# neuromodulation/PyPARRM

Hardware: NVIDIA B200
Metric: filter_data channel-samples/sec (higher is better)
Workload: dtype f64

## Files before the change

pyparrm_b200/csrc/filter.cu:

```cuda
#include <string.h>

#include "common.cuh"
#include "filter_jit.h"
#include "filter_plan.h"
#include "gather.cuh"

namespace parrm {

static thread_local const char* g_last_kernel = "";

template <typename T>
struct FilterArgs {
  const T* x;
  T* out;
  const int32_t* taps;
  int64_t ld_x, x_t0, n_x;
  int64_t ld_out, t0, n_out;
  int64_t n_total;
  int32_t n_taps, w_lo, w_hi;
  int32_t tile;
};

template <typename T>
__global__ void __launch_bounds__(kGatherThreads)
// ... 109 lines not shown
  filter_gather_smem_kernel<T><<<grid, kGatherThreads, smem, stream>>>(a);
  PARRM_LAUNCH_OK("filter_gather_smem_kernel");
  g_last_kernel = "filter_gather_smem_kernel";
  return PARRM_OK;
}


}

extern "C" {

const char* parrm_filter_last_kernel(void) { return parrm::g_last_kernel; }

int parrm_filter_specialise_check(const void* h_plan, int dtype,
                                  const parrm_filter_options_t* options, int32_t* shape,
                                  size_t* cubin_bytes) {
  using namespace parrm;
  PARRM_REQUIRE(h_plan != nullptr, "parrm_filter_specialise_check: null plan");
  const FilterPlanHeader* hdr = static_cast<const FilterPlanHeader*>(h_plan);
  PARRM_REQUIRE(hdr->magic == kPlanMagic && hdr->version == kPlanVersion,
                "parrm_filter_specialise_check: not a filter plan");
  const int32_t* h_terms = reinterpret_cast<const int32_t*>(
      static_cast<const unsigned char*>(h_plan) + hdr->terms_offset);
  FilterTuning tune{0, options ? options->steps_per_chunk : 0,
                    options ? options->prefetch_chunks : 0, options ? options->ctas_per_sm : 0,
                    options ? options->variant : 0, options ? options->timeline : 0};
  CombEShape s;
  if (!comb_e_shape(hdr, h_terms, dtype, &tune, &s)) {
    set_error("parrm_filter_specialise_check: this plan is outside the specialised kernel's range");
    return PARRM_ERR_UNSUPPORTED;
  }
  if (shape) {
    const int32_t v[12] = {s.d, s.nk, s.m[0], s.m[1], s.nb[0], s.nb[1], s.n_plus + s.n_minus,
                           s.u, s.pf, s.ctas, s.smem_bytes, ((s.d + 31) / 32) * 32 + 32};
    for (int i = 0; i < 12; ++i) shape[i] = v[i];
  }
  if (cubin_bytes == nullptr) return PARRM_OK;
  return comb_e_compile_only(s, cubin_bytes);
}

int parrm_filter_apply(const void* d_x, int64_t ld_x, int64_t x_t0, int64_t n_x, void* d_out,
                       int64_t ld_out, int64_t t0, int64_t n_out, int64_t n_samples_total,
                       int64_t n_chans, const void* d_plan, const void* h_plan, int dtype,
                       void* stream) {
  return parrm_filter_apply_ex(d_x, ld_x, x_t0, n_x, d_out, ld_out, t0, n_out, n_samples_total,
                               n_chans, d_plan, h_plan, dtype, nullptr, stream);
}

int parrm_filter_apply_ex(const void* d_x, int64_t ld_x, int64_t x_t0, int64_t n_x, void* d_out,
                          int64_t ld_out, int64_t t0, int64_t n_out, int64_t n_samples_total,
                          int64_t n_chans, const void* d_plan, const void* h_plan, int dtype,
                          const parrm_filter_options_t* options, void* stream) {
  PARRM_NVTX("parrm_filter_apply_ex");
  using namespace parrm;
  PARRM_REQUIRE(d_plan != nullptr && h_plan != nullptr, "parrm_filter_apply: null plan");
  const FilterPlanHeader* hdr = static_cast<const FilterPlanHeader*>(h_plan);
  PARRM_REQUIRE(hdr->magic == kPlanMagic && hdr->version == kPlanVersion,
                "parrm_filter_apply: not a filter plan");
  PARRM_REQUIRE(hdr->dtype == dtype, "parrm_filter_apply: plan built for another dtype");
  PARRM_REQUIRE(dtype == PARRM_F64 || dtype == PARRM_F32, "parrm_filter_apply: bad dtype %d", dtype);
  PARRM_REQUIRE(n_chans >= 0 && n_out >= 0 && n_x >= 0 && n_samples_total >= 0,
                "parrm_filter_apply: negative size");
  PARRM_REQUIRE(n_chans <= 65535, "parrm_filter_apply: more than 65535 channels per call");
  const int want = options ? options->kernel : PARRM_FILTER_KERNEL_AUTO;
  PARRM_REQUIRE(want == PARRM_FILTER_KERNEL_AUTO || want == PARRM_FILTER_KERNEL_GATHER ||
                    want == PARRM_FILTER_KERNEL_SPECIALISED,
                "parrm_filter_apply: unknown kernel choice %d", want);
// ... 101 lines not shown
```

pyparrm_b200/csrc/filter_comb_e.cuh:

```cuda
#pragma once

#ifdef __CUDACC_RTC__
typedef signed char int8_t;
typedef int int32_t;
typedef unsigned int uint32_t;
typedef long long int64_t;
typedef unsigned long long uint64_t;
typedef unsigned long long uintptr_t;
#else
#include <stdint.h>
#endif

#ifndef PE_D
#define PE_T double
#define PE_D 200
#define PE_NK 2
#define PE_M0 20
#define PE_M1 10
#define PE_NB0 7
#define PE_NB1 2
#define PE_OFF0 -1969, -1954, -1923, -1877, -1846, -1831, -1800
#define PE_OFF1 -1908, 108
#define PE_NPLUS 1
#define PE_PLUS -2000
#define PE_NMINUS 0
#define PE_MINUS 0
#define PE_CENTRE -1
#define PE_U 10
#define PE_PF 2
#define PE_NTAPS 160
#define PE_WLO -2000
#define PE_WHI 2000
#define PE_BACK 108
#define PE_FWD 2000
#define PE_CTAS 2
#endif
#ifndef PE_VARIANT
#define PE_VARIANT 0
#endif

namespace parrm_e {

typedef PE_T T;
typedef double T2;
constexpr int D = PE_D;
constexpr int NK = PE_NK;
constexpr int M0 = PE_M0;
constexpr int M1 = PE_M1;
constexpr int NB0 = PE_NB0;
constexpr int NB1 = PE_NB1;
constexpr int NPLUS = PE_NPLUS;
constexpr int NMINUS = PE_NMINUS;
constexpr int CENTRE = PE_CENTRE;
constexpr int U = PE_U;
constexpr int PF = PE_PF;
constexpr int NTAPS = PE_NTAPS;
constexpr int WLO = PE_WLO;
constexpr int WHI = PE_WHI;
constexpr int BACK = PE_BACK;
constexpr int FWD = PE_FWD;
constexpr int ES = int(sizeof(T));
constexpr int VEC = 16 / ES;
constexpr int CH = U * D;
constexpr int HB = (BACK + CH - 1) / CH;
constexpr int HF = (FWD + CH - 1) / CH;
constexpr int MIR = HB + HF;
constexpr int Q = HB + HF + 1 + PF;
constexpr int GPB = (M0 + U - 1) / U;
constexpr int B = GPB * U;
constexpr int NPG = GPB;
constexpr int NW = (D + 31) / 32;
constexpr int NT = NW * 32 + 32;
constexpr int BAR_BYTES = ((2 * Q * 8 + 127) / 128) * 128;
constexpr int SMEM_BYTES = BAR_BYTES + (Q + MIR) * CH * ES;
static_assert((CH * ES) % 16 == 0, "chunk must be a whole number of 16-byte units");
static_assert(M0 >= M1 && M0 >= 1, "box lengths ordered");

__host__ __device__ constexpr int off0(int b) {
  constexpr int t[NB0 > 0 ? NB0 : 1] = {PE_OFF0};
  return t[b];
}
__host__ __device__ constexpr int off1(int b) {
  constexpr int t[NB1 > 0 ? NB1 : 1] = {PE_OFF1};
  return t[b];
}
__host__ __device__ constexpr int plus_tap(int i) {
  constexpr int t[NPLUS > 0 ? NPLUS : 1] = {PE_PLUS};
  return t[i];
}
__host__ __device__ constexpr int minus_tap(int i) {
  constexpr int t[NMINUS > 0 ? NMINUS : 1] = {PE_MINUS};
  return t[i];
}

struct Args {
  const T* x;
  T* out;
  const int32_t* taps;
  const int32_t* count;
  const T2* recip;
  int64_t ld_x, x_t0, n_x;
  int64_t ld_out, t0, n_out;
  int64_t n_total;
  int64_t total_groups;
  int32_t groups_per_chan;
// ... 53 lines not shown
                                        T xc, T tot) {
  const int64_t v1 = min64(max64(t, WLO - 1), WHI);
  const int64_t v2 = min64(max64(t - n_total, WLO - 1), WHI);
  const int n_in = count[v1 - (WLO - 1)] - count[v2 - (WLO - 1)];
  T y = xc - tot * T(recip[n_in]);
  if (n_in == 0) y = T(0);
  return y;
}

__device__ __noinline__ T direct_value(const int32_t* __restrict__ taps,
                                       const T2* __restrict__ recip, int64_t n_total, T t_max,
                                       const T* __restrict__ xrow, int64_t t, int64_t lo_valid,
                                       int64_t hi_valid) {
  T acc = T(0);
  int n_in = 0;
  for (int k = 0; k < NTAPS; ++k) {
    const int64_t g = t - taps[k];
    if (g < 0 || g >= n_total) continue;
    ++n_in;
    if (g >= lo_valid && g < hi_valid) acc += xrow[g];
  }
  if (n_in == 0) return T(0);
  const T y = xrow[t] - acc * T(recip[n_in]);
  return fabs(y) <= t_max ? y : T(0);
}

struct Walk {
  int pb;
  int rslot;
  int fslot;
  uint32_t fphase;
};

__device__ __forceinline__ void group_begin(Walk& w, uint32_t bars) {
  mbar_wait(bars + w.fslot * 8, w.fphase);
  if (++w.fslot == Q) {
    w.fslot = 0;
    w.fphase ^= 1u;
  }
}
__device__ __forceinline__ void group_end(Walk& w, uint32_t bars, int lane, unsigned wmask) {
  __syncwarp(wmask);
  if (lane == 0) {
    asm volatile("mbarrier.arrive.shared::cta.b64 _, [%0];" ::"r"(bars + (Q + w.rslot) * 8)
                 : "memory");
  }
  w.pb += CH * ES;
  if (++w.rslot == Q) {
    w.rslot = 0;
    w.pb -= Q * CH * ES;
  }
}

struct Rings {
  T r0[B];
  T r1[NK > 1 ? B : 1];
  T S0, S1;
};

__device__ __forceinline__ T ring_sum0(const Rings& r, int s) {
  T a = r.r0[s];
#pragma unroll
  for (int i = 1; i < M0; ++i) a += r.r0[(s + B - i) % B];
  return a;
}
__device__ __forceinline__ T ring_sum1(const Rings& r, int s) {
  if (NK < 2) return T(0);
  T a = r.r1[s];
#pragma unroll
  for (int i = 1; i < M1; ++i) a += r.r1[(s + B - i) % B];
  return a;
}

template <bool FAST>
__device__ __forceinline__ int run_block(Rings& r, Walk& w, const Args& a,
                                         const unsigned char* const smem, uint32_t bars,
                                         int lane, unsigned wmask, int c, T* const orow,
                                         int& bad_lo, int& bad_hi, int64_t Tb, int g,
                                         int n_groups) {
  const T neg_inv_n = a.neg_inv_n;
  const T t_max = a.t_max;
  T* const op = orow + Tb + c;
  int done = 0;
#pragma unroll
  for (int gi = 0; gi < GPB; ++gi) {
    if (!FAST && g + gi >= n_groups) break;
    group_begin(w, bars);
    int mode = 1;
    if (!FAST) {
      const int64_t Tn = Tb + int64_t(gi) * CH;
      const bool interior = (Tn - WHI >= 0) && (Tn + CH - WLO <= a.n_total);
      const bool all_out = (Tn >= a.t0) && (Tn + CH <= a.t0 + a.n_out);
      mode = (g + gi < NPG) ? 0 : ((interior && all_out) ? 1 : 2);
    }
    const unsigned char* const p = smem + w.pb;
#pragma unroll
    for (int js = 0; js < U; ++js) {
      const int s = gi * U + js;
      auto ld = [&](int off) {
        return *reinterpret_cast<const T*>(p + (HB * CH + js * D - off) * ES);
      };
      r.S0 -= r.r0[(s + B - M0) % B];
      if (NK > 1) r.S1 -= r.r1[(s + B - M1) % B];
      T e0 = ld(off0(0));
      if (NB0 > 1) {
        T e0b = ld(off0(1));
#pragma unroll
        for (int b = 2; b < NB0; ++b) {
          if (b & 1) e0b += ld(off0(b)); else e0 += ld(off0(b));
        }
        e0 += e0b;
      }
      r.r0[s] = e0;
      r.S0 += e0;
      T tot = r.S0;
      if (NK > 1) {
        T e1 = ld(off1(0));
        if (NB1 > 1) {
          T e1b = ld(off1(1));
#pragma unroll
          for (int b = 2; b < NB1; ++b) {
            if (b & 1) e1b += ld(off1(b)); else e1 += ld(off1(b));
          }
          e1 += e1b;
        }
        r.r1[s] = e1;
        r.S1 += e1;
        tot += r.S1;
      }
      T single = T(0);
      if (NPLUS > 0) {
        single = ld(plus_tap(0));
#pragma unroll
        for (int i = 1; i < NPLUS; ++i) single += ld(plus_tap(i));
      }
#pragma unroll
      for (int i = 0; i < NMINUS; ++i) single -= ld(minus_tap(i));
      const T xc = ld(0);
      if (CENTRE != 0) single = fma(T(CENTRE), xc, single);
      if (NPLUS > 0 || NMINUS > 0 || CENTRE != 0) tot += single;
      if (FAST) {
        T y = fma(tot, neg_inv_n, xc);
        if (__builtin_expect(!(fabs(y) <= t_max), 0)) {
          r.S0 = ring_sum0(r, s);
          r.S1 = ring_sum1(r, s);
          bad_lo = min(bad_lo, g * U + s);
          bad_hi = max(bad_hi, g * U + s);
          y = T(0);
        }
        op[s * D] = y;
      } else if (mode != 0) {
        const int64_t t = Tb + c + int64_t(s) * D;
        if (ES == 4 && mode == 2) {
          r.S0 = ring_sum0(r, s);
          r.S1 = ring_sum1(r, s);
          tot = r.S0;
          if (NK > 1) tot += r.S1;
          if (NPLUS > 0 || NMINUS > 0 || CENTRE != 0) tot += single;
        }
        T y = mode == 1 ? fma(tot, neg_inv_n, xc) : edge_value(a.count, a.recip, t, a.n_total, xc, tot);
        if (__builtin_expect(!(fabs(y) <= t_max), 0)) {
          r.S0 = ring_sum0(r, s);
          r.S1 = ring_sum1(r, s);
          bad_lo = min(bad_lo, g * U + s);
          bad_hi = max(bad_hi, g * U + s);
          y = T(0);
        }
        if (t >= a.t0 && t < a.t0 + a.n_out) op[s * D] = y;
      }
    }
    group_end(w, bars, lane, wmask);
    ++done;
  }
  return done;
}

extern "C" __global__ void __launch_bounds__(NT, PE_CTAS) parrm_filter_comb_e(const Args a) {
  extern __shared__ __align__(128) unsigned char smem_raw[];
  uint64_t* const full = reinterpret_cast<uint64_t*>(smem_raw);
  uint64_t* const empty = full + Q;
  T* const ring = reinterpret_cast<T*>(smem_raw + BAR_BYTES);
  const int tid = threadIdx.x;
  const int lane = tid & 31;
  const bool is_producer = tid >= NW * 32;

  if (tid == 0) {
    for (int s = 0; s < Q; ++s) {
      mbar_init(&full[s], 1);
      mbar_init(&empty[s], NW);
    }
    asm volatile("fence.mbarrier_init.release.cluster;" ::: "memory");
  }
  __syncthreads();

  const int64_t lo_valid = max64(0, a.x_t0);
  const int64_t hi_valid = min64(a.n_total, a.x_t0 + a.n_x);
#if PE_VARIANT & 2
  unsigned long long tl_start = 0, tl_pieces = 0;
  if (tid == 0) asm volatile("mov.u64 %0, %%globaltimer;" : "=l"(tl_start));
#endif
  const int gpc = a.groups_per_chan;
  const int vpc = gpc + a.edge_total;
  const int64_t G_begin = a.total_groups * int64_t(blockIdx.x) / int64_t(gridDim.x);
  const int64_t G_end = a.total_groups * int64_t(blockIdx.x + 1) / int64_t(gridDim.x);
  const uint32_t bars = smem_u32(smem_raw);

  int fslot = 0;
  uint32_t fphase = 0;
  int rslot = 0;

  for (int64_t G = G_begin; G < G_end;) {
    const int64_t chan = G / vpc;
    const int v0 = int(G - chan * vpc);
    const int v1 = int(min64(vpc, v0 + (G_end - G)));
    G += v1 - v0;
    const int s0 = min(max(v0 - a.edge_start, 0), gpc);
    const int s1 = min(max(v1 - a.edge_start, 0), gpc);
    if (s1 <= s0) continue;
    const T* const xrow = a.x + chan * a.ld_x - a.x_t0;
    T* const orow = a.out + chan * a.ld_out - a.t0;
    const int gamma = int((VEC - int((reinterpret_cast<uintptr_t>(xrow) / ES) % VEC)) % VEC);
    const int64_t j_first = floor_div(a.t0 - gamma, CH);
    const int64_t j_last = floor_div(a.t0 + a.n_out - 1 - gamma, CH);
    const int64_t n_first = j_first + s0;
    const int64_t n_end = min64(j_first + s1, j_last + 1);
    if (n_first >= n_end) continue;
#if PE_VARIANT & 2
    ++tl_pieces;
#endif
    const int n_groups = NPG + int(n_end - n_first);
    const int n_chunks = n_groups + HB + HF;
    const int64_t c_first = n_first - NPG - HB;

    if (is_producer) {
      for (int i = 0; i < n_chunks; ++i) {
        const int64_t g0 = gamma + (c_first + i) * int64_t(CH);
        T* const dst = ring + fslot * CH;
        mbar_wait(bars + (Q + fslot) * 8, fphase ^ 1u);
        if (g0 >= lo_valid && g0 + CH <= hi_valid) {
          if (lane == 0) {
            asm volatile("fence.proxy.async.shared::cta;" ::: "memory");
            const bool mirror = fslot < MIR;
            mbar_expect_tx(&full[fslot], uint32_t(CH * ES) * (mirror ? 2u : 1u));
            bulk_g2s(dst, xrow + g0, uint32_t(CH * ES), &full[fslot]);
            if (mirror) bulk_g2s(dst + Q * CH, xrow + g0, uint32_t(CH * ES), &full[fslot]);
          }
        } else {
          for (int e = lane; e < CH; e += 32) {
            const int64_t g = g0 + e;
            const T v = (g >= lo_valid && g < hi_valid) ? xrow[g] : T(0);
            dst[e] = v;
            if (fslot < MIR) dst[Q * CH + e] = v;
          }
          __syncwarp();
          if (lane == 0) mbar_arrive(&full[fslot]);
        }
        if (++fslot == Q) {
          fslot = 0;
          fphase ^= 1u;
        }
      }
      continue;
    }

    if (tid >= D) continue;
    const int c = tid;
    const unsigned wmask = (tid | 31) < D ? 0xffffffffu : ((1u << (D & 31)) - 1u);
    for (int i = 0; i < HB + HF; ++i) {
      mbar_wait(bars + fslot * 8, fphase);
      if (++fslot == Q) {
        fslot = 0;
        fphase ^= 1u;
      }
    }
    Rings r;
#pragma unroll
    for (int s = 0; s < B; ++s) r.r0[s] = T(0);
#pragma unroll
    for (int s = 0; s < (NK > 1 ? B : 1); ++s) r.r1[s] = T(0);
    const int64_t T0 = gamma + (n_first - NPG) * int64_t(CH);
    Walk w;
    w.pb = BAR_BYTES + (rslot * CH + c) * ES;
    w.rslot = rslot;
    w.fslot = fslot;
    w.fphase = fphase;
    int bad_lo = 1 << 30, bad_hi = -1;
    for (int g = 0; g < n_groups;) {
      const int64_t Tb = T0 + int64_t(g) * CH;
      r.S0 = ring_sum0(r, B - 1);
      r.S1 = ring_sum1(r, B - 1);
      const bool fast = g >= NPG && g + GPB <= n_groups && Tb - WHI >= 0 &&
                        Tb + int64_t(B) * D - WLO <= a.n_total && Tb >= a.t0 &&
                        Tb + int64_t(B) * D <= a.t0 + a.n_out;
      if (fast) {
        g += run_block<true>(r, w, a, smem_raw, bars, lane, wmask, c, orow, bad_lo, bad_hi,
                             Tb, g, n_groups);
      } else {
        g += run_block<false>(r, w, a, smem_raw, bars, lane, wmask, c, orow, bad_lo, bad_hi,
                              Tb, g, n_groups);
      }
    }
    rslot = w.rslot;
    fslot = w.fslot;
    fphase = w.fphase;
    for (int k = bad_lo; k <= bad_hi; ++k) {
      const int64_t t = T0 + c + int64_t(k) * D;
      if (t >= a.t0 && t < a.t0 + a.n_out)
        orow[t] = direct_value(a.taps, a.recip, a.n_total, a.t_max, xrow, t, lo_valid, hi_valid);
    }
    __syncwarp(wmask);
    for (int i = 0; i < HB + HF; ++i) {
      if (lane == 0) mbar_arrive(&empty[rslot]);
      if (++rslot == Q) rslot = 0;
    }
  }
#if PE_VARIANT & 2
  if (tid == 0 && a.timeline) {
    unsigned long long tl_end;
    unsigned smid;
    asm volatile("mov.u64 %0, %%globaltimer;" : "=l"(tl_end));
    asm volatile("mov.u32 %0, %%smid;" : "=r"(smid));
    a.timeline[4 * blockIdx.x + 0] = smid;
    a.timeline[4 * blockIdx.x + 1] = tl_start;
    a.timeline[4 * blockIdx.x + 2] = tl_end;
    a.timeline[4 * blockIdx.x + 3] = tl_pieces;
  }
#endif
}

}
```

pyparrm_b200/csrc/filter_jit.cu:

```cuda
#include <cuda.h>
#include <dlfcn.h>
#include <string.h>

#include <algorithm>
#include <map>
#include <mutex>
#include <string>
#include <vector>

#include "common.cuh"
#include "filter_jit.h"
#include "filter_plan.h"

namespace parrm {
namespace {

const char kCombESource[] =
#include "filter_comb_e_src.inc"
    ;

typedef struct _nvrtcProgram* nvrtcProgram;
struct Nvrtc {
  void* handle = nullptr;
  int (*CreateProgram)(nvrtcProgram*, const char*, const char*, int, const char* const*,
// ... 150 lines not shown
    const int64_t ch = int64_t(u) * s.d;
    const int64_t hb = (s.back + ch - 1) / ch, hf = (s.fwd + ch - 1) / ch;
    const int64_t q = hb + hf + 1 + pf;
    return ((2 * q * 8 + 127) / 128) * 128 + (q + hb + hf) * ch * s.es;
  };
  auto usable = [&](int u) {
    return u >= 1 && (int64_t(u) * s.d * s.es) % 16 == 0 && (s.m[0] + u - 1) / u * u <= 64;
  };
  for (int ctas = ctas_first; ctas >= 1; --ctas) {
    const int64_t budget = int64_t(227) * 1024 / ctas - 1024;
    int u = 0;
    if (tune && tune->steps_per_chunk > 0) {
      u = tune->steps_per_chunk;
      if (!usable(u) || smem_for(u, pf_min) > budget) u = 0;
    } else {
      for (int cand = s.m[0]; cand >= 1 && u == 0; --cand)
        if (s.m[0] % cand == 0 && int64_t(cand) * s.d * s.es <= 32768 &&
            int64_t(cand) * s.d >= 512 && usable(cand) && smem_for(cand, pf_min) <= budget)
          u = cand;
      const int u_hi = int(std::max<int64_t>(1, 20480 / (int64_t(s.d) * s.es)));
      for (int cand = u_hi; cand >= 1 && u == 0; --cand)
        if (usable(cand) && smem_for(cand, pf_min) <= budget) u = cand;
      for (int cand = 1; cand <= 64 && u == 0; ++cand)
        if (usable(cand) && smem_for(cand, pf_min) <= budget) u = cand;
    }
    if (u == 0) continue;
    int pf = pf_min;
    while (pf < pf_max && smem_for(u, pf + 1) <= budget) ++pf;
    s.smem_bytes = int(smem_for(u, pf));
    s.ctas = ctas;
    s.u = u;
    s.pf = pf;
    s.variant = tune ? tune->variant : 0;
    *out = s;
    return true;
  }
  return false;
}

static int compile_cubin(const CombEShape& s, std::vector<char>* cubin) {
  Nvrtc* n = nvrtc();
  if (!n->ok) {
    const char* why = dlerror();
    set_error("parrm filter: NVRTC (libnvrtc.so.12) could not be opened: %s", why ? why : "?");
    return PARRM_ERR_UNSUPPORTED;
  }
  std::vector<std::string> opts = {
      "--gpu-architecture=sm_100a", "-std=c++17", "-lineinfo",
      std::string("-DPE_T=") + (s.es == 8 ? "double" : "float"),
      "-DPE_D=" + std::to_string(s.d), "-DPE_NK=" + std::to_string(s.nk),
      "-DPE_M0=" + std::to_string(s.m[0]), "-DPE_M1=" + std::to_string(s.m[1]),
      "-DPE_NB0=" + std::to_string(s.nb[0]), "-DPE_NB1=" + std::to_string(s.nb[1]),
      "-DPE_OFF0=" + join(s.off[0], s.nb[0]), "-DPE_OFF1=" + join(s.off[1], s.nb[1]),
      "-DPE_NPLUS=" + std::to_string(s.n_plus), "-DPE_PLUS=" + join(s.plus, s.n_plus),
      "-DPE_NMINUS=" + std::to_string(s.n_minus), "-DPE_MINUS=" + join(s.minus, s.n_minus),
      "-DPE_CENTRE=" + std::to_string(s.centre), "-DPE_U=" + std::to_string(s.u),
      "-DPE_PF=" + std::to_string(s.pf), "-DPE_NTAPS=" + std::to_string(s.n_taps),
      "-DPE_WLO=" + std::to_string(s.w_lo), "-DPE_WHI=" + std::to_string(s.w_hi),
      "-DPE_BACK=" + std::to_string(s.back), "-DPE_FWD=" + std::to_string(s.fwd),
      "-DPE_CTAS=" + std::to_string(s.ctas), "-DPE_VARIANT=" + std::to_string(s.variant)};
  std::vector<const char*> copts;
  for (const std::string& o : opts) copts.push_back(o.c_str());
  nvrtcProgram prog = nullptr;
  int rc = n->CreateProgram(&prog, kCombESource, "filter_comb_e.cu", 0, nullptr, nullptr);
  if (rc != 0) {
    set_error("nvrtcCreateProgram: %s", n->GetErrorString(rc));
    return PARRM_ERR_CUDA;
  }
  rc = n->CompileProgram(prog, int(copts.size()), copts.data());
  if (rc != 0) {
    size_t log_size = 0;
    n->GetProgramLogSize(prog, &log_size);
    std::string log(log_size + 1, '\0');
    if (log_size) n->GetProgramLog(prog, &log[0]);
    set_error("nvrtcCompileProgram: %s\n%.380s", n->GetErrorString(rc), log.c_str());
    n->DestroyProgram(&prog);
    return PARRM_ERR_CUDA;
  }
  size_t cubin_size = 0;
  n->GetCUBINSize(prog, &cubin_size);
  cubin->resize(cubin_size);
  rc = n->GetCUBIN(prog, cubin->data());
  n->DestroyProgram(&prog);
  if (rc != 0 || cubin_size == 0) {
    set_error("nvrtcGetCUBIN: %s", n->GetErrorString(rc));
    return PARRM_ERR_CUDA;
  }
  return PARRM_OK;
}

int comb_e_compile_only(const CombEShape& s, size_t* cubin_bytes) {
  std::vector<char> cubin;
  const int rc = compile_cubin(s, &cubin);
  if (rc == PARRM_OK && cubin_bytes) *cubin_bytes = cubin.size();
  return rc;
}

static int build_kernel(const CombEShape& s, Kernel* out) {
  Driver* d = driver();
  if (!d->ok) {
    set_error("parrm filter: CUDA driver entry points unavailable");
    return PARRM_ERR_UNSUPPORTED;
  }
  std::vector<char> cubin;
  const int rc = compile_cubin(s, &cubin);
  if (rc != PARRM_OK) return rc;
  PARRM_CUDA_OK(cudaFree(nullptr));
  CUmodule mod = nullptr;
  CUresult cr = d->ModuleLoadData(&mod, cubin.data());
  if (cr != CUDA_SUCCESS) return driver_fail(cr, "cuModuleLoadData");
  Kernel k;
  cr = d->ModuleGetFunction(&k.fn, mod, "parrm_filter_comb_e");
  if (cr != CUDA_SUCCESS) return driver_fail(cr, "cuModuleGetFunction");
  k.smem_bytes = s.smem_bytes;
  k.threads = ((s.d + 31) / 32) * 32 + 32;
  k.ctas_per_sm = s.ctas;
  k.chunk = s.u * s.d;
  k.priming_groups = (s.m[0] + s.u - 1) / s.u;
  cr = d->FuncSetAttribute(k.fn, CU_FUNC_ATTRIBUTE_MAX_DYNAMIC_SHARED_SIZE_BYTES, k.smem_bytes);
  if (cr != CUDA_SUCCESS) return driver_fail(cr, "cuFuncSetAttribute(max dynamic shared memory)");
  d->FuncSetAttribute(k.fn, CU_FUNC_ATTRIBUTE_PREFERRED_SHARED_MEMORY_CARVEOUT, 100);
  d->FuncGetAttribute(&k.regs, CU_FUNC_ATTRIBUTE_NUM_REGS, k.fn);
  *out = k;
  return PARRM_OK;
}

bool comb_e_cached(const CombEShape& s) {
  int dev = 0;
  if (cudaGetDevice(&dev) != cudaSuccess) return false;
  const std::string key = comb_e_key(s, dev);
  std::lock_guard<std::mutex> lock(g_mutex);
  return g_cache.count(key) != 0;
}

std::string comb_e_key(const CombEShape& s, int dev) {
  std::string key = std::to_string(dev) + "|" + std::to_string(s.es) + "|" + std::to_string(s.d) +
                    "|" + std::to_string(s.nk) + "|" + std::to_string(s.m[0]) + "|" +
                    std::to_string(s.m[1]) + "|" + join(s.off[0], s.nb[0]) + "|" +
                    join(s.off[1], s.nb[1]) + "|" + join(s.plus, s.n_plus) + "|" +
                    join(s.minus, s.n_minus) + "|" + std::to_string(s.centre) + "|" +
                    std::to_string(s.u) + "|" + std::to_string(s.pf) + "|" +
                    std::to_string(s.n_taps) + "|" + std::to_string(s.w_lo) + "|" +
                    std::to_string(s.w_hi) + "|" + std::to_string(s.ctas) + "|" +
                    std::to_string(s.variant);
  return key;
}

int launch_comb_e(const CombEShape& s, const void* d_x, void* d_out, const int32_t* d_taps,
                  const int32_t* d_count, const double* d_recip,
                  int64_t ld_x, int64_t x_t0, int64_t n_x, int64_t ld_out, int64_t t0,
                  int64_t n_out, int64_t n_total, int64_t n_chans, cudaStream_t stream,
                  int* regs_out, unsigned long long timeline) {
  int dev = 0;
  PARRM_CUDA_OK(cudaGetDevice(&dev));
  const std::string key = comb_e_key(s, dev);
  Kernel k;
  {
    std::lock_guard<std::mutex> lock(g_mutex);
    auto it = g_cache.find(key);
    if (it == g_cache.end()) {
      const int rc = build_kernel(s, &k);
      if (rc != PARRM_OK) return rc;
      g_cache[key] = k;
    } else {
      k = it->second;
    }
  }
  if (regs_out) *regs_out = k.regs;
  struct Args {
    const void* x;
    void* out;
    const int32_t* taps;
    const int32_t* count;
    const double* recip;
    int64_t ld_x, x_t0, n_x, ld_out, t0, n_out, n_total, total_groups;
    int32_t groups_per_chan, edge_start, edge_total, pad;
    unsigned long long timeline;
// ... 35 lines not shown
```

pyparrm_b200/csrc/filter_jit.h:

```cpp
#pragma once
#include <cuda_runtime.h>
#include <stdint.h>

#include <string>

#include "filter_plan.h"

namespace parrm {

struct FilterTuning {
  int kernel;
  int steps_per_chunk;
  int prefetch_chunks;
  int ctas_per_sm;
  int variant;
  unsigned long long timeline;
};

struct CombEShape {
  int es;
  int d, nk, m[2], nb[2];
  const int32_t* off[2];
  int n_plus, n_minus;
  const int32_t *plus, *minus;
  int centre, n_taps, w_lo, w_hi, back, fwd;
  int u, pf, ctas, smem_bytes, variant;
};

bool comb_e_shape(const FilterPlanHeader* hdr, const int32_t* terms, int dtype,
                  const FilterTuning* tune, CombEShape* out);
std::string comb_e_key(const CombEShape& s, int dev);
bool comb_e_cached(const CombEShape& s);
int comb_e_compile_only(const CombEShape& s, size_t* cubin_bytes);
int launch_comb_e(const CombEShape& s, const void* d_x, void* d_out, const int32_t* d_taps,
                  const int32_t* d_count, const double* d_recip,
                  int64_t ld_x, int64_t x_t0, int64_t n_x, int64_t ld_out, int64_t t0,
                  int64_t n_out, int64_t n_total, int64_t n_chans, cudaStream_t stream,
                  int* regs_out, unsigned long long timeline = 0);

}
```

pyparrm_b200/csrc/filter_plan.cu:

```cuda
#include <algorithm>
#include <string.h>
#include <vector>

#include "common.cuh"
#include "filter_plan.h"

namespace parrm {
namespace {

struct CombPlan {
  int d = 0, nk = 0;
  int m[kMaxBoxKinds] = {0, 0};
  std::vector<int> box[kMaxBoxKinds];
  std::vector<int> plus, minus;
  int centre = 0;
  double cost = 1e30;
  int n_terms() const { return int(box[0].size() + box[1].size() + plus.size() + minus.size()); }
};

bool cover(const std::vector<uint8_t>& bit, int lo, int hi, int d, int nk, const int* m,
           CombPlan* out) {
  const int span = hi - lo + 1;
  CombPlan p;
  p.d = d;
// ... 127 lines not shown
    std::vector<int> cand;
    auto add_len = [&](int len) {
      if (len >= 2 && len <= max_ring && std::find(cand.begin(), cand.end(), len) == cand.end())
        cand.push_back(len);
    };
    for (size_t i = 0; i < lengths.size() && i < 6; ++i) add_len(lengths[i].second);
    for (size_t i = 0; i < lengths.size() && i < 3 && cand.size() < 8; ++i) {
      const int len = lengths[i].second;
      if (len > max_ring || 2 * len > max_ring) {
        add_len((len + 1) / 2);
        add_len((len + 2) / 3);
      }
    }
    const int n_len = int(cand.size());
    for (int i = 0; i < n_len; ++i) {
      for (int j = i; j < n_len; ++j) {
        int m[2] = {cand[i], cand[j]};
        if (i != j && m[0] + m[1] > max_ring) continue;
        CombPlan p;
        if (!cover(bit, lo, hi, d, i == j ? 1 : 2, m, &p)) continue;
        if (p.n_terms() > kMaxTerms) continue;
        const int ring = p.m[0] + (p.nk > 1 ? p.m[1] : 0);
        if (ring > max_ring) continue;
        p.cost = double(p.n_terms()) + 1e-3 * ring;
        if (p.cost < best->cost) {
          *best = p;
          found = true;
        }
      }
    }
  }
  if (!found) return false;
  return exact(*best, bit, lo, hi);
}

}
}

extern "C" {

static size_t plan_layout(const int32_t* h_taps, int32_t n_taps, size_t* recip_off, size_t* count_off) {
  const size_t n = size_t(n_taps > 0 ? n_taps : 0);
  size_t off = sizeof(parrm::FilterPlanHeader) + (n + parrm::kMaxTerms) * sizeof(int32_t);
  off = (off + 7) & ~size_t(7);
  if (recip_off) *recip_off = off;
  off += (n + 1) * sizeof(double);
  if (count_off) *count_off = off;
  int64_t span = 0;
  if (n > 0 && h_taps != nullptr) {
    const int64_t lo = h_taps[0] < 0 ? h_taps[0] : 0;
    const int64_t hi = h_taps[n - 1] > 0 ? h_taps[n - 1] : 0;
    span = hi - lo;
  }
  off += size_t(span + 2) * sizeof(int32_t);
  return (off + 15) & ~size_t(15);
}

size_t parrm_filter_plan_bytes(const int32_t* h_taps, int32_t n_taps) {
  return plan_layout(h_taps, n_taps, nullptr, nullptr);
}

int parrm_filter_plan(const int32_t* h_taps, int32_t n_taps, int dtype, int strategy,
                      void* h_plan, size_t plan_bytes) {
  using namespace parrm;
  PARRM_REQUIRE(n_taps > 0 && h_taps != nullptr, "parrm_filter_plan: empty tap list");
  PARRM_REQUIRE(h_plan != nullptr, "parrm_filter_plan: null plan buffer");
// ... 40 lines not shown
    }
  }
  if (strategy == PARRM_PLAN_GATHER) return PARRM_OK;

  CombPlan best;
  const bool ok = best_comb(h_taps, n_taps, kPatternFirstMinStride, kPatternFirstMaxStride,
                            dtype == PARRM_F64 ? 8 : 4, &best);
  const bool worth = ok && (strategy == PARRM_PLAN_COMB || best.cost < 0.6 * double(n_taps));
  if (!worth) {
    if (strategy == PARRM_PLAN_COMB) {
      set_error("parrm_filter_plan: this tap set has no comb structure");
      return PARRM_ERR_UNSUPPORTED;
    }
    return PARRM_OK;
  }
  hdr->kind = kPlanComb;
  hdr->stride = best.d;
  hdr->n_kinds = best.nk;
  int32_t* terms = reinterpret_cast<int32_t*>(base + hdr->terms_offset);
  int n = 0;
  for (int k = 0; k < best.nk; ++k) {
    hdr->window[k] = best.m[k];
    hdr->n_box[k] = int32_t(best.box[k].size());
    hdr->a_min[k] = best.box[k].front();
    hdr->a_max[k] = best.box[k].back();
    for (int a : best.box[k]) terms[n++] = a;
  }
  hdr->n_plus = int32_t(best.plus.size());
  hdr->n_minus = int32_t(best.minus.size());
  for (int w : best.plus) terms[n++] = w;
  for (int w : best.minus) terms[n++] = w;
  hdr->centre = best.centre;
  hdr->cost_milli = int32_t(best.cost * 1000.0);
  return PARRM_OK;
}

}

extern "C" int parrm_filter_plan_info(const void* h_plan, int32_t* info, int32_t* terms,
                                      int32_t capacity) {
  using namespace parrm;
  PARRM_REQUIRE(h_plan != nullptr && info != nullptr, "parrm_filter_plan_info: null pointer");
  const FilterPlanHeader* hdr = static_cast<const FilterPlanHeader*>(h_plan);
  PARRM_REQUIRE(hdr->magic == kPlanMagic && hdr->version == kPlanVersion,
                "parrm_filter_plan_info: not a filter plan");
  const int32_t n_terms = hdr->kind == kPlanComb
                              ? hdr->n_box[0] + hdr->n_box[1] + hdr->n_plus + hdr->n_minus
                              : 0;
  const int32_t v[16] = {hdr->kind, hdr->stride, hdr->n_kinds, hdr->window[0], hdr->window[1],
                         hdr->n_box[0], hdr->n_box[1], hdr->n_plus, hdr->n_minus, hdr->centre,
                         hdr->cost_milli, hdr->n_taps, hdr->w_min, hdr->w_max, n_terms, 0};
  for (int i = 0; i < 16; ++i) info[i] = v[i];
  if (terms != nullptr) {
    PARRM_REQUIRE(capacity >= n_terms, "parrm_filter_plan_info: terms buffer too small");
    const int32_t* src = reinterpret_cast<const int32_t*>(
        static_cast<const unsigned char*>(h_plan) + hdr->terms_offset);
    for (int i = 0; i < n_terms; ++i) terms[i] = src[i];
  }
  return PARRM_OK;
}
```

pyparrm_b200/csrc/filter_plan.h:

```cpp
#pragma once
#include <stdint.h>

namespace parrm {

constexpr uint32_t kPlanMagic = 0x4D525250u;
constexpr uint32_t kPlanVersion = 4;
constexpr int kMaxTerms = 120;
constexpr int kMaxBoxKinds = 2;

enum PlanKind : int32_t {
  kPlanGather = 0,
  kPlanComb = 1
};

struct FilterPlanHeader {
  uint32_t magic;
  uint32_t version;
  int32_t n_taps;
  int32_t w_min, w_max;
  int32_t kind;
  int32_t taps_offset;
  int32_t dtype;
  int32_t stride;
  int32_t n_kinds;
  int32_t window[kMaxBoxKinds];
  int32_t n_box[kMaxBoxKinds];
  int32_t a_min[kMaxBoxKinds];
  int32_t a_max[kMaxBoxKinds];
  int32_t n_plus, n_minus;
  int32_t centre;
  int32_t terms_offset;
  int32_t cost_milli;
  int32_t count_offset;
  int32_t recip_offset;
  int32_t total_bytes;
  int32_t reserved[6];
};
static_assert(sizeof(FilterPlanHeader) == 128, "plan header is 128 bytes");

constexpr int kPatternFirstMinStride = 64;
constexpr int kPatternFirstMaxStride = 992;
constexpr int kPatternFirstMaxRing = 60;
constexpr int kPatternFirstStepRegs = 52;

inline int pattern_first_threads(int d) { return ((d + 31) / 32) * 32 + 32; }
inline int pattern_first_reg_budget(int d, int ctas) {
  const int r = (65536 / (ctas * pattern_first_threads(d))) / 8 * 8;
  return r < 255 ? r : 255;
}
inline int pattern_first_max_ring(int d, int es) {
  const int ring = (pattern_first_reg_budget(d, 1) - kPatternFirstStepRegs) / (es / 4);
  return ring < kPatternFirstMaxRing ? ring : kPatternFirstMaxRing;
}

}
```

Baseline: 309.1 billion.

## Pair two columns per consumer thread to share shared-memory loads in comb kernel

Adds a paired mode in which each consumer thread processes two columns a fixed distance apart. The distance is picked when the plan is built so that many tap loads of the second column hit the same addresses as the first, cutting the number of distinct shared-memory loads per output sample. Consumers become a single 128-thread warpgroup and producers give registers back through setmaxnreg, so each consumer can hold two sets of ring registers. The costs are extra register pressure, a fixed 256-thread launch shape, and new plan and JIT fields, and the mode applies only to f64 with two CTAs per SM.

```diff
diff --git a/pyparrm_b200/csrc/filter.cu b/pyparrm_b200/csrc/filter.cu
--- a/pyparrm_b200/csrc/filter.cu
+++ b/pyparrm_b200/csrc/filter.cu
@@ -165,7 +165,7 @@
   }
   if (shape) {
     const int32_t v[12] = {s.d, s.nk, s.m[0], s.m[1], s.nb[0], s.nb[1], s.n_plus + s.n_minus,
-                           s.u, s.pf, s.ctas, s.smem_bytes, ((s.d + 31) / 32) * 32 + 32};
+                           s.u, s.pf, s.ctas, s.smem_bytes, s.threads};
     for (int i = 0; i < 12; ++i) shape[i] = v[i];
   }
   if (cubin_bytes == nullptr) return PARRM_OK;
diff --git a/pyparrm_b200/csrc/filter_comb_e.cuh b/pyparrm_b200/csrc/filter_comb_e.cuh
--- a/pyparrm_b200/csrc/filter_comb_e.cuh
+++ b/pyparrm_b200/csrc/filter_comb_e.cuh
@@ -34,6 +34,7 @@
 #define PE_BACK 108
 #define PE_FWD 2000
 #define PE_CTAS 2
+#define PE_PAIR 46
 #endif
 #ifndef PE_VARIANT
 #define PE_VARIANT 0
@@ -69,8 +70,19 @@
 constexpr int GPB = (M0 + U - 1) / U;
 constexpr int B = GPB * U;
 constexpr int NPG = GPB;
-constexpr int NW = (D + 31) / 32;
-constexpr int NT = NW * 32 + 32;
+constexpr int PAIR = PE_PAIR;
+constexpr int LB = PAIR > 0 ? (PAIR + 128 / ES - 1) / (128 / ES) * (128 / ES) : 1;
+constexpr int NBLK = PAIR > 0 ? D / (2 * PAIR) : 0;
+constexpr int NPAIRED = NBLK * PAIR;
+constexpr int NSINGLE = D - 2 * NPAIRED;
+constexpr int WP = (NBLK * LB + 31) / 32;
+constexpr int NW = WP + (NSINGLE + 31) / 32;
+constexpr int NCT = PAIR > 0 ? 128 : NW * 32;
+constexpr int NT = NCT + (PAIR > 0 ? 128 : 32);
+constexpr int REG_PRODUCER = 24;
+constexpr int REG_CONSUMER = (65536 / PE_CTAS / 128 - REG_PRODUCER) / 8 * 8;
+static_assert(PAIR == 0 || (NBLK > 0 && NW <= 4 && PE_CTAS == 2),
+              "paired CTA: one consumer warpgroup at two CTAs per SM");
 constexpr int BAR_BYTES = ((2 * Q * 8 + 127) / 128) * 128;
 constexpr int SMEM_BYTES = BAR_BYTES + (Q + MIR) * CH * ES;
 static_assert((CH * ES) % 16 == 0, "chunk must be a whole number of 16-byte units");
@@ -190,6 +202,10 @@
   uint32_t fphase;
 };
 
+__device__ __forceinline__ void mbar_release(uint32_t bars, int slot) {
+  asm volatile("mbarrier.arrive.shared::cta.b64 _, [%0];" ::"r"(bars + (Q + slot) * 8) : "memory");
+}
+
 __device__ __forceinline__ void group_begin(Walk& w, uint32_t bars) {
   mbar_wait(bars + w.fslot * 8, w.fphase);
   if (++w.fslot == Q) {
@@ -199,10 +215,7 @@
 }
 __device__ __forceinline__ void group_end(Walk& w, uint32_t bars, int lane, unsigned wmask) {
   __syncwarp(wmask);
-  if (lane == 0) {
-    asm volatile("mbarrier.arrive.shared::cta.b64 _, [%0];" ::"r"(bars + (Q + w.rslot) * 8)
-                 : "memory");
-  }
+  if (lane == 0) mbar_release(bars, w.rslot);
   w.pb += CH * ES;
   if (++w.rslot == Q) {
     w.rslot = 0;
@@ -230,11 +243,11 @@
   return a;
 }
 
-template <bool FAST>
-__device__ __forceinline__ int run_block(Rings& r, Walk& w, const Args& a,
+template <bool FAST, int NC>
+__device__ __forceinline__ int run_block(Rings (&r)[NC], Walk& w, const Args& a,
                                          const unsigned char* const smem, uint32_t bars,
                                          int lane, unsigned wmask, int c, T* const orow,
-                                         int& bad_lo, int& bad_hi, int64_t Tb, int g,
+                                         int (&bad_lo)[NC], int (&bad_hi)[NC], int64_t Tb, int g,
                                          int n_groups) {
   const T neg_inv_n = a.neg_inv_n;
   const T t_max = a.t_max;
@@ -255,76 +268,84 @@
 #pragma unroll
     for (int js = 0; js < U; ++js) {
       const int s = gi * U + js;
-      auto ld = [&](int off) {
-        return *reinterpret_cast<const T*>(p + (HB * CH + js * D - off) * ES);
-      };
-      r.S0 -= r.r0[(s + B - M0) % B];
-      if (NK > 1) r.S1 -= r.r1[(s + B - M1) % B];
-      T e0 = ld(off0(0));
-      if (NB0 > 1) {
-        T e0b = ld(off0(1));
-#pragma unroll
-        for (int b = 2; b < NB0; ++b) {
-          if (b & 1) e0b += ld(off0(b)); else e0 += ld(off0(b));
-        }
-        e0 += e0b;
+      T yk[NC];
+#pragma unroll
+      for (int k = 0; k < NC; ++k) {
+        Rings& rk = r[k];
+        auto ld = [&](int off) {
+          return *reinterpret_cast<const T*>(p + (HB * CH + js * D + k * PAIR - off) * ES);
+        };
+        rk.S0 -= rk.r0[(s + B - M0) % B];
+        if (NK > 1) rk.S1 -= rk.r1[(s + B - M1) % B];
+        T e0 = ld(off0(0));
+        if (NB0 > 1) {
+          T e0b = ld(off0(1));
+#pragma unroll
+          for (int b = 2; b < NB0; ++b) {
+            if (b & 1) e0b += ld(off0(b)); else e0 += ld(off0(b));
+          }
+          e0 += e0b;
+        }
+        rk.r0[s] = e0;
+        rk.S0 += e0;
+        T tot = rk.S0;
+        if (NK > 1) {
+          T e1 = ld(off1(0));
+          if (NB1 > 1) {
+            T e1b = ld(off1(1));
+#pragma unroll
+            for (int b = 2; b < NB1; ++b) {
+              if (b & 1) e1b += ld(off1(b)); else e1 += ld(off1(b));
+            }
+            e1 += e1b;
+          }
+          rk.r1[s] = e1;
+          rk.S1 += e1;
+          tot += rk.S1;
+        }
+        T single = T(0);
+        if (NPLUS > 0) {
+          single = ld(plus_tap(0));
+#pragma unroll
+          for (int i = 1; i < NPLUS; ++i) single += ld(plus_tap(i));
+        }
+#pragma unroll
+        for (int i = 0; i < NMINUS; ++i) single -= ld(minus_tap(i));
+        const T xc = ld(0);
+        if (CENTRE != 0) single = fma(T(CENTRE), xc, single);
+        if (NPLUS > 0 || NMINUS > 0 || CENTRE != 0) tot += single;
+        T y = T(0);
+        if (FAST) {
+          y = fma(tot, neg_inv_n, xc);
+        } else if (mode != 0) {
+          const int64_t t = Tb + c + k * PAIR + int64_t(s) * D;
+          if (ES == 4 && mode == 2) {
+            rk.S0 = ring_sum0(rk, s);
+            rk.S1 = ring_sum1(rk, s);
+            tot = rk.S0;
+            if (NK > 1) tot += rk.S1;
+            if (NPLUS > 0 || NMINUS > 0 || CENTRE != 0) tot += single;
+          }
+          y = mode == 1 ? fma(tot, neg_inv_n, xc)
+                        : edge_value(a.count, a.recip, t, a.n_total, xc, tot);
+        }
+        if ((FAST || mode != 0) && __builtin_expect(!(fabs(y) <= t_max), 0)) {
+          rk.S0 = ring_sum0(rk, s);
+          rk.S1 = ring_sum1(rk, s);
+          bad_lo[k] = min(bad_lo[k], g * U + s);
+          bad_hi[k] = max(bad_hi[k], g * U + s);
+          y = T(0);
+        }
+        yk[k] = y;
       }
-      r.r0[s] = e0;
-      r.S0 += e0;
-      T tot = r.S0;
-      if (NK > 1) {
-        T e1 = ld(off1(0));
-        if (NB1 > 1) {
-          T e1b = ld(off1(1));
-#pragma unroll
-          for (int b = 2; b < NB1; ++b) {
-            if (b & 1) e1b += ld(off1(b)); else e1 += ld(off1(b));
-          }
-          e1 += e1b;
-        }
-        r.r1[s] = e1;
-        r.S1 += e1;
-        tot += r.S1;
-      }
-      T single = T(0);
-      if (NPLUS > 0) {
-        single = ld(plus_tap(0));
-#pragma unroll
-        for (int i = 1; i < NPLUS; ++i) single += ld(plus_tap(i));
-      }
-#pragma unroll
-      for (int i = 0; i < NMINUS; ++i) single -= ld(minus_tap(i));
-      const T xc = ld(0);
-      if (CENTRE != 0) single = fma(T(CENTRE), xc, single);
-      if (NPLUS > 0 || NMINUS > 0 || CENTRE != 0) tot += single;
-      if (FAST) {
-        T y = fma(tot, neg_inv_n, xc);
-        if (__builtin_expect(!(fabs(y) <= t_max), 0)) {
-          r.S0 = ring_sum0(r, s);
-          r.S1 = ring_sum1(r, s);
-          bad_lo = min(bad_lo, g * U + s);
-          bad_hi = max(bad_hi, g * U + s);
-          y = T(0);
-        }
-        op[s * D] = y;
-      } else if (mode != 0) {
-        const int64_t t = Tb + c + int64_t(s) * D;
-        if (ES == 4 && mode == 2) {
-          r.S0 = ring_sum0(r, s);
-          r.S1 = ring_sum1(r, s);
-          tot = r.S0;
-          if (NK > 1) tot += r.S1;
-          if (NPLUS > 0 || NMINUS > 0 || CENTRE != 0) tot += single;
-        }
-        T y = mode == 1 ? fma(tot, neg_inv_n, xc) : edge_value(a.count, a.recip, t, a.n_total, xc, tot);
-        if (__builtin_expect(!(fabs(y) <= t_max), 0)) {
-          r.S0 = ring_sum0(r, s);
-          r.S1 = ring_sum1(r, s);
-          bad_lo = min(bad_lo, g * U + s);
-          bad_hi = max(bad_hi, g * U + s);
-          y = T(0);
-        }
-        if (t >= a.t0 && t < a.t0 + a.n_out) op[s * D] = y;
+#pragma unroll
+      for (int k = 0; k < NC; ++k) {
+        if (FAST) {
+          op[s * D + k * PAIR] = yk[k];
+        } else if (mode != 0) {
+          const int64_t t = Tb + c + k * PAIR + int64_t(s) * D;
+          if (t >= a.t0 && t < a.t0 + a.n_out) op[s * D + k * PAIR] = yk[k];
+        }
       }
     }
     group_end(w, bars, lane, wmask);
@@ -333,40 +354,79 @@
   return done;
 }
 
-extern "C" __global__ void __launch_bounds__(NT, PE_CTAS) parrm_filter_comb_e(const Args a) {
-  extern __shared__ __align__(128) unsigned char smem_raw[];
-  uint64_t* const full = reinterpret_cast<uint64_t*>(smem_raw);
-  uint64_t* const empty = full + Q;
-  T* const ring = reinterpret_cast<T*>(smem_raw + BAR_BYTES);
-  const int tid = threadIdx.x;
-  const int lane = tid & 31;
-  const bool is_producer = tid >= NW * 32;
-
-  if (tid == 0) {
-    for (int s = 0; s < Q; ++s) {
-      mbar_init(&full[s], 1);
-      mbar_init(&empty[s], NW);
-    }
-    asm volatile("fence.mbarrier_init.release.cluster;" ::: "memory");
-  }
-  __syncthreads();
-
-  const int64_t lo_valid = max64(0, a.x_t0);
-  const int64_t hi_valid = min64(a.n_total, a.x_t0 + a.n_x);
-#if PE_VARIANT & 2
-  unsigned long long tl_start = 0, tl_pieces = 0;
-  if (tid == 0) asm volatile("mov.u64 %0, %%globaltimer;" : "=l"(tl_start));
-#endif
+template <int NC>
+__device__ __forceinline__ void run_piece(const Args& a, const unsigned char* const smem,
+                                          uint32_t bars, int lane, unsigned wmask, int c,
+                                          const T* const xrow, T* const orow, int64_t T0,
+                                          int n_groups, int64_t lo_valid, int64_t hi_valid,
+                                          int& rslot, int& fslot, uint32_t& fphase) {
+  for (int i = 0; i < HB + HF; ++i) {
+    mbar_wait(bars + fslot * 8, fphase);
+    if (++fslot == Q) {
+      fslot = 0;
+      fphase ^= 1u;
+    }
+  }
+  Rings r[NC];
+#pragma unroll
+  for (int k = 0; k < NC; ++k) {
+#pragma unroll
+    for (int s = 0; s < B; ++s) r[k].r0[s] = T(0);
+#pragma unroll
+    for (int s = 0; s < (NK > 1 ? B : 1); ++s) r[k].r1[s] = T(0);
+  }
+  Walk w;
+  w.pb = BAR_BYTES + (rslot * CH + c) * ES;
+  w.rslot = rslot;
+  w.fslot = fslot;
+  w.fphase = fphase;
+  int bad_lo[NC], bad_hi[NC];
+#pragma unroll
+  for (int k = 0; k < NC; ++k) {
+    bad_lo[k] = 1 << 30;
+    bad_hi[k] = -1;
+  }
+  for (int g = 0; g < n_groups;) {
+    const int64_t Tb = T0 + int64_t(g) * CH;
+#pragma unroll
+    for (int k = 0; k < NC; ++k) {
+      r[k].S0 = ring_sum0(r[k], B - 1);
+      r[k].S1 = ring_sum1(r[k], B - 1);
+    }
+    const bool fast = g >= NPG && g + GPB <= n_groups && Tb - WHI >= 0 &&
+                      Tb + int64_t(B) * D - WLO <= a.n_total && Tb >= a.t0 &&
+                      Tb + int64_t(B) * D <= a.t0 + a.n_out;
+    if (fast) {
+      g += run_block<true, NC>(r, w, a, smem, bars, lane, wmask, c, orow, bad_lo, bad_hi, Tb, g,
+                               n_groups);
+    } else {
+      g += run_block<false, NC>(r, w, a, smem, bars, lane, wmask, c, orow, bad_lo, bad_hi, Tb, g,
+                                n_groups);
+    }
+  }
+  rslot = w.rslot;
+  fslot = w.fslot;
+  fphase = w.fphase;
+#pragma unroll
+  for (int k = 0; k < NC; ++k) {
+    for (int j = bad_lo[k]; j <= bad_hi[k]; ++j) {
+      const int64_t t = T0 + c + k * PAIR + int64_t(j) * D;
+      if (t >= a.t0 && t < a.t0 + a.n_out)
+        orow[t] = direct_value(a.taps, a.recip, a.n_total, a.t_max, xrow, t, lo_valid, hi_valid);
+    }
+  }
+  __syncwarp(wmask);
+  for (int i = 0; i < HB + HF; ++i) {
+    if (lane == 0) mbar_release(bars, rslot);
+    if (++rslot == Q) rslot = 0;
+  }
+}
+
+template <class F>
+__device__ __forceinline__ void for_each_piece(const Args& a, int64_t G_begin, int64_t G_end,
+                                               F&& piece) {
   const int gpc = a.groups_per_chan;
   const int vpc = gpc + a.edge_total;
-  const int64_t G_begin = a.total_groups * int64_t(blockIdx.x) / int64_t(gridDim.x);
-  const int64_t G_end = a.total_groups * int64_t(blockIdx.x + 1) / int64_t(gridDim.x);
-  const uint32_t bars = smem_u32(smem_raw);
-
-  int fslot = 0;
-  uint32_t fphase = 0;
-  int rslot = 0;
-
   for (int64_t G = G_begin; G < G_end;) {
     const int64_t chan = G / vpc;
     const int v0 = int(G - chan * vpc);
@@ -383,14 +443,60 @@
     const int64_t n_first = j_first + s0;
     const int64_t n_end = min64(j_first + s1, j_last + 1);
     if (n_first >= n_end) continue;
+    piece(xrow, orow, gamma, n_first, NPG + int(n_end - n_first));
+  }
+}
+
+extern "C" __global__ void __launch_bounds__(NT, PE_CTAS) parrm_filter_comb_e(const Args a) {
+  extern __shared__ __align__(128) unsigned char smem_raw[];
+  uint64_t* const full = reinterpret_cast<uint64_t*>(smem_raw);
+  uint64_t* const empty = full + Q;
+  T* const ring = reinterpret_cast<T*>(smem_raw + BAR_BYTES);
+  const int tid = threadIdx.x;
+  const int lane = tid & 31;
+  const bool is_producer = tid >= NCT;
+  const bool paired = PAIR > 0 && tid < WP * 32;
+  int c = tid;
+  bool active = tid < D;
+  if (paired) {
+    const int blk = tid / LB, i = tid % LB;
+    c = 2 * PAIR * blk + i;
+    active = blk < NBLK && i < PAIR;
+  } else if (PAIR > 0) {
+    c = 2 * NPAIRED + tid - WP * 32;
+    active = c < D;
+  }
+
+  if (tid == 0) {
+    for (int s = 0; s < Q; ++s) {
+      mbar_init(&full[s], 1);
+      mbar_init(&empty[s], NW);
+    }
+    asm volatile("fence.mbarrier_init.release.cluster;" ::: "memory");
+  }
+  __syncthreads();
+  const int64_t lo_valid = max64(0, a.x_t0);
+  const int64_t hi_valid = min64(a.n_total, a.x_t0 + a.n_x);
 #if PE_VARIANT & 2
-    ++tl_pieces;
+  unsigned long long tl_start = 0, tl_pieces = 0;
+  if (tid == 0) asm volatile("mov.u64 %0, %%globaltimer;" : "=l"(tl_start));
 #endif
-    const int n_groups = NPG + int(n_end - n_first);
-    const int n_chunks = n_groups + HB + HF;
-    const int64_t c_first = n_first - NPG - HB;
-
-    if (is_producer) {
+  const int64_t G_begin = a.total_groups * int64_t(blockIdx.x) / int64_t(gridDim.x);
+  const int64_t G_end = a.total_groups * int64_t(blockIdx.x + 1) / int64_t(gridDim.x);
+  const uint32_t bars = smem_u32(smem_raw);
+
+  int fslot = 0;
+  uint32_t fphase = 0;
+  int rslot = 0;
+
+  if (is_producer) {
+    if constexpr (PAIR > 0) {
+      asm volatile("setmaxnreg.dec.sync.aligned.u32 %0;" ::"n"(REG_PRODUCER));
+      if (tid >= NCT + 32) return;
+    }
+    for_each_piece(a, G_begin, G_end, [&](const T* xrow, T*, int gamma, int64_t n_first, int n_groups) {
+      const int n_chunks = n_groups + HB + HF;
+      const int64_t c_first = n_first - NPG - HB;
       for (int i = 0; i < n_chunks; ++i) {
         const int64_t g0 = gamma + (c_first + i) * int64_t(CH);
         T* const dst = ring + fslot * CH;
@@ -418,60 +524,29 @@
           fphase ^= 1u;
         }
       }
-      continue;
-    }
-
-    if (tid >= D) continue;
-    const int c = tid;
-    const unsigned wmask = (tid | 31) < D ? 0xffffffffu : ((1u << (D & 31)) - 1u);
-    for (int i = 0; i < HB + HF; ++i) {
-      mbar_wait(bars + fslot * 8, fphase);
-      if (++fslot == Q) {
-        fslot = 0;
-        fphase ^= 1u;
+    });
+    return;
+  }
+
+  if constexpr (PAIR > 0) asm volatile("setmaxnreg.inc.sync.aligned.u32 %0;" ::"n"(REG_CONSUMER));
+  const unsigned wmask = __ballot_sync(0xffffffffu, active);
+  if (!active) return;
+  for_each_piece(a, G_begin, G_end, [&](const T* xrow, T* orow, int gamma, int64_t n_first,
+                                         int n_groups) {
+#if PE_VARIANT & 2
+    ++tl_pieces;
+#endif
+    const int64_t T0 = gamma + (n_first - NPG) * int64_t(CH);
+    if constexpr (PAIR > 0) {
+      if (paired) {
+        run_piece<2>(a, smem_raw, bars, lane, wmask, c, xrow, orow, T0, n_groups, lo_valid,
+                     hi_valid, rslot, fslot, fphase);
+        return;
       }
     }
-    Rings r;
-#pragma unroll
-    for (int s = 0; s < B; ++s) r.r0[s] = T(0);
-#pragma unroll
-    for (int s = 0; s < (NK > 1 ? B : 1); ++s) r.r1[s] = T(0);
-    const int64_t T0 = gamma + (n_first - NPG) * int64_t(CH);
-    Walk w;
-    w.pb = BAR_BYTES + (rslot * CH + c) * ES;
-    w.rslot = rslot;
-    w.fslot = fslot;
-    w.fphase = fphase;
-    int bad_lo = 1 << 30, bad_hi = -1;
-    for (int g = 0; g < n_groups;) {
-      const int64_t Tb = T0 + int64_t(g) * CH;
-      r.S0 = ring_sum0(r, B - 1);
-      r.S1 = ring_sum1(r, B - 1);
-      const bool fast = g >= NPG && g + GPB <= n_groups && Tb - WHI >= 0 &&
-                        Tb + int64_t(B) * D - WLO <= a.n_total && Tb >= a.t0 &&
-                        Tb + int64_t(B) * D <= a.t0 + a.n_out;
-      if (fast) {
-        g += run_block<true>(r, w, a, smem_raw, bars, lane, wmask, c, orow, bad_lo, bad_hi,
-                             Tb, g, n_groups);
-      } else {
-        g += run_block<false>(r, w, a, smem_raw, bars, lane, wmask, c, orow, bad_lo, bad_hi,
-                              Tb, g, n_groups);
-      }
-    }
-    rslot = w.rslot;
-    fslot = w.fslot;
-    fphase = w.fphase;
-    for (int k = bad_lo; k <= bad_hi; ++k) {
-      const int64_t t = T0 + c + int64_t(k) * D;
-      if (t >= a.t0 && t < a.t0 + a.n_out)
-        orow[t] = direct_value(a.taps, a.recip, a.n_total, a.t_max, xrow, t, lo_valid, hi_valid);
-    }
-    __syncwarp(wmask);
-    for (int i = 0; i < HB + HF; ++i) {
-      if (lane == 0) mbar_arrive(&empty[rslot]);
-      if (++rslot == Q) rslot = 0;
-    }
-  }
+    run_piece<1>(a, smem_raw, bars, lane, wmask, c, xrow, orow, T0, n_groups, lo_valid, hi_valid,
+                 rslot, fslot, fphase);
+  });
 #if PE_VARIANT & 2
   if (tid == 0 && a.timeline) {
     unsigned long long tl_end;
diff --git a/pyparrm_b200/csrc/filter_jit.cu b/pyparrm_b200/csrc/filter_jit.cu
--- a/pyparrm_b200/csrc/filter_jit.cu
+++ b/pyparrm_b200/csrc/filter_jit.cu
@@ -206,6 +206,11 @@
     s.u = u;
     s.pf = pf;
     s.variant = tune ? tune->variant : 0;
+    s.pair = ctas == 2 && !(s.variant & 8) && pattern_first_pair_fits(s.d, hdr->pair, s.m[0] + (s.nk > 1 ? s.m[1] : 0),
+                                                  s.es)
+                 ? hdr->pair
+                 : 0;
+    s.threads = s.pair ? 256 : threads;
     *out = s;
     return true;
   }
@@ -232,7 +237,8 @@
       "-DPE_PF=" + std::to_string(s.pf), "-DPE_NTAPS=" + std::to_string(s.n_taps),
       "-DPE_WLO=" + std::to_string(s.w_lo), "-DPE_WHI=" + std::to_string(s.w_hi),
       "-DPE_BACK=" + std::to_string(s.back), "-DPE_FWD=" + std::to_string(s.fwd),
-      "-DPE_CTAS=" + std::to_string(s.ctas), "-DPE_VARIANT=" + std::to_string(s.variant)};
+      "-DPE_CTAS=" + std::to_string(s.ctas), "-DPE_VARIANT=" + std::to_string(s.variant),
+      "-DPE_PAIR=" + std::to_string(s.pair)};
   std::vector<const char*> copts;
   for (const std::string& o : opts) copts.push_back(o.c_str());
   nvrtcProgram prog = nullptr;
@@ -287,7 +293,7 @@
   cr = d->ModuleGetFunction(&k.fn, mod, "parrm_filter_comb_e");
   if (cr != CUDA_SUCCESS) return driver_fail(cr, "cuModuleGetFunction");
   k.smem_bytes = s.smem_bytes;
-  k.threads = ((s.d + 31) / 32) * 32 + 32;
+  k.threads = s.threads;
   k.ctas_per_sm = s.ctas;
   k.chunk = s.u * s.d;
   k.priming_groups = (s.m[0] + s.u - 1) / s.u;
@@ -316,7 +322,7 @@
                     std::to_string(s.u) + "|" + std::to_string(s.pf) + "|" +
                     std::to_string(s.n_taps) + "|" + std::to_string(s.w_lo) + "|" +
                     std::to_string(s.w_hi) + "|" + std::to_string(s.ctas) + "|" +
-                    std::to_string(s.variant);
+                    std::to_string(s.variant) + "|" + std::to_string(s.pair);
   return key;
 }
 
diff --git a/pyparrm_b200/csrc/filter_jit.h b/pyparrm_b200/csrc/filter_jit.h
--- a/pyparrm_b200/csrc/filter_jit.h
+++ b/pyparrm_b200/csrc/filter_jit.h
@@ -25,6 +25,8 @@
   const int32_t *plus, *minus;
   int centre, n_taps, w_lo, w_hi, back, fwd;
   int u, pf, ctas, smem_bytes, variant;
+  int pair;
+  int threads;
 };
 
 bool comb_e_shape(const FilterPlanHeader* hdr, const int32_t* terms, int dtype,
diff --git a/pyparrm_b200/csrc/filter_plan.cu b/pyparrm_b200/csrc/filter_plan.cu
--- a/pyparrm_b200/csrc/filter_plan.cu
+++ b/pyparrm_b200/csrc/filter_plan.cu
@@ -183,6 +183,41 @@
   }
   if (!found) return false;
   return exact(*best, bit, lo, hi);
+}
+
+int step_loads(const CombPlan& p, int delta) {
+  std::vector<int> off;
+  for (int k = 0; k < p.nk; ++k) off.insert(off.end(), p.box[k].begin(), p.box[k].end());
+  off.insert(off.end(), p.plus.begin(), p.plus.end());
+  off.insert(off.end(), p.minus.begin(), p.minus.end());
+  off.push_back(0);
+  std::vector<int> all(off);
+  if (delta > 0)
+    for (int v : off) all.push_back(v - delta);
+  std::sort(all.begin(), all.end());
+  all.erase(std::unique(all.begin(), all.end()), all.end());
+  int n = 0;
+  for (int v : all)
+    if (!std::binary_search(all.begin(), all.end(), v - p.d)) ++n;
+  return n;
+}
+
+int choose_pair(const CombPlan& p, int es) {
+  const int ring = p.m[0] + (p.nk > 1 ? p.m[1] : 0);
+  const int single = step_loads(p, 0);
+  int best = 0;
+  int64_t best_milli = int64_t(single) * 1000;
+  for (int delta = 1; 2 * delta <= p.d; ++delta) {
+    if (!pattern_first_pair_fits(p.d, delta, ring, es)) continue;
+    const int paired = p.d / (2 * delta) * delta;
+    const int64_t milli =
+        (int64_t(paired) * step_loads(p, delta) + int64_t(p.d - 2 * paired) * single) * 1000 / p.d;
+    if (milli < best_milli) {
+      best_milli = milli;
+      best = delta;
+    }
+  }
+  return best_milli * 10 <= int64_t(single) * 1000 * 9 ? best : 0;
 }
 
 }
@@ -289,6 +324,7 @@
   for (int w : best.minus) terms[n++] = w;
   hdr->centre = best.centre;
   hdr->cost_milli = int32_t(best.cost * 1000.0);
+  hdr->pair = choose_pair(best, dtype == PARRM_F64 ? 8 : 4);
   return PARRM_OK;
 }
 
@@ -306,7 +342,7 @@
                               : 0;
   const int32_t v[16] = {hdr->kind, hdr->stride, hdr->n_kinds, hdr->window[0], hdr->window[1],
                          hdr->n_box[0], hdr->n_box[1], hdr->n_plus, hdr->n_minus, hdr->centre,
-                         hdr->cost_milli, hdr->n_taps, hdr->w_min, hdr->w_max, n_terms, 0};
+                         hdr->cost_milli, hdr->n_taps, hdr->w_min, hdr->w_max, n_terms, hdr->pair};
   for (int i = 0; i < 16; ++i) info[i] = v[i];
   if (terms != nullptr) {
     PARRM_REQUIRE(capacity >= n_terms, "parrm_filter_plan_info: terms buffer too small");
diff --git a/pyparrm_b200/csrc/filter_plan.h b/pyparrm_b200/csrc/filter_plan.h
--- a/pyparrm_b200/csrc/filter_plan.h
+++ b/pyparrm_b200/csrc/filter_plan.h
@@ -34,7 +34,8 @@
   int32_t count_offset;
   int32_t recip_offset;
   int32_t total_bytes;
-  int32_t reserved[6];
+  int32_t pair;
+  int32_t reserved[5];
 };
 static_assert(sizeof(FilterPlanHeader) == 128, "plan header is 128 bytes");
 
@@ -53,4 +54,21 @@
   return ring < kPatternFirstMaxRing ? ring : kPatternFirstMaxRing;
 }
 
+constexpr int kPairConsumerRegs = 232;
+constexpr int kPairStepRegs = 80;
+inline int pattern_first_pair_lanes(int delta, int es) {
+  const int g = 128 / es;
+  return (delta + g - 1) / g * g;
 }
+inline int pattern_first_pair_threads(int d, int delta, int es) {
+  const int blocks = d / (2 * delta);
+  const int single = d - 2 * blocks * delta;
+  return (blocks * pattern_first_pair_lanes(delta, es) + 31) / 32 * 32 + (single + 31) / 32 * 32;
+}
+inline bool pattern_first_pair_fits(int d, int delta, int ring, int es) {
+  return es == 8 && delta >= 1 && 2 * delta <= d &&
+         pattern_first_pair_threads(d, delta, es) <= 128 &&
+         2 * ring * (es / 4) + kPairStepRegs <= kPairConsumerRegs;
+}
+
+}
```

New measurement: 154.0 billion (median of 6 runs). -50.2%, worse.
